# Seasandwpy/viso

Measured on AMD Instinct MI355X. Metric: stereo frames/sec at 1242x375 grey, 1/2/4/8 GPUs; pose RMSE vs reference, higher is better.
Workload: dtype f64

## Files before the change

### viso_amd/csrc/common.hpp

```cpp
#pragma once

#include <hip/hip_runtime.h>

#include <cstddef>
#include <cstdint>
#include <cstdio>

namespace viso {

constexpr int kLevels = 4;
constexpr int kHalfPatch = 4;
constexpr int kPatch = 64;
constexpr int kMaxWidth = 4096;

struct PyrGeom {
    int w[kLevels], h[kLevels];
    size_t off[kLevels];
    size_t bytes;
    size_t slot;
};

inline PyrGeom make_geom(int w, int h) {
    PyrGeom g{};
    size_t off = 0;
// ... 36 lines not shown
    return ((const __attribute__((address_space(1))) uint8_t*)p)[i];
}
__device__ inline uint8_t ld_global_u8_off(const uint8_t* base, uint32_t off) {
    return ((const __attribute__((address_space(1))) uint8_t*)base)[off];
}
__device__ inline int ld_u8_or0(const uint8_t* p, long long n, long long i) {
    const bool in = i >= 0 && i < n;
    const int v = ld_global_u8(p, in ? i : 0);
    return in ? v : 0;
}
__device__ inline uint8_t ld_lds_u8(const uint8_t* p, int i) {
    return ((const __attribute__((address_space(3))) uint8_t*)p)[i];
}
__device__ inline void st_lds_u8(uint8_t* p, int i, uint8_t v) {
    ((__attribute__((address_space(3))) uint8_t*)p)[i] = v;
}

__device__ inline double sample_px(const uint8_t* __restrict__ img, int w, int h, double x,
                                   double y) {
    const long long n = (long long)w * (long long)h;
    const bool finite = (x > -1e9 && x < 1e9 && y > -1e9 && y < 1e9);
    long long base = finite ? (long long)(int)y * (long long)w + (long long)(int)x : -(1LL << 40);
    double d0 = (double)ld_u8_or0(img, n, base);
    double d1 = (double)ld_u8_or0(img, n, base + 1);
    double d2 = (double)ld_u8_or0(img, n, base + w);
    double d3 = (double)ld_u8_or0(img, n, base + w + 1);
    double xx = x - floor(x);
    double yy = y - floor(y);
    return double((1 - xx) * (1 - yy) * d0 + xx * (1 - yy) * d1 + (1 - xx) * yy * d2 +
                  xx * yy * d3);
}

__device__ inline void gradient_px(const uint8_t* __restrict__ img, int w, int h, double u,
                                   double v, double& gx, double& gy) {
    gx = 0.5 * (sample_px(img, w, h, u + 1, v) - sample_px(img, w, h, u - 1, v));
    gy = 0.5 * (sample_px(img, w, h, u, v + 1) - sample_px(img, w, h, u, v - 1));
}

__device__ inline double wave_tree_sum(double v) {
#pragma unroll
    for (int off = 1; off < 64; off <<= 1) v = v + __shfl_xor(v, off, 64);
    return v;
}

template <int CTRL>
__device__ inline double dpp_f64(double v) {
    const long long b = __double_as_longlong(v);
    const int lo = __builtin_amdgcn_mov_dpp((int)(b & 0xffffffffLL), CTRL, 0xF, 0xF, true);
    const int hi = __builtin_amdgcn_mov_dpp((int)(b >> 32), CTRL, 0xF, 0xF, true);
    return __longlong_as_double(((long long)hi << 32) | (unsigned int)lo);
}

__device__ inline int wave_id() { return __builtin_amdgcn_readfirstlane((int)(threadIdx.x >> 6)); }

__device__ inline double uniform_f64(double v) {
    const long long b = __double_as_longlong(v);
    const int lo = __builtin_amdgcn_readfirstlane((int)(b & 0xffffffffLL));
    const int hi = __builtin_amdgcn_readfirstlane((int)(b >> 32));
    return __longlong_as_double(((long long)hi << 32) | (unsigned int)lo);
}

__device__ inline double readlane_f64(double v, int lane) {
    const long long b = __double_as_longlong(v);
    const int lo = __builtin_amdgcn_readlane((int)(b & 0xffffffffLL), lane);
    const int hi = __builtin_amdgcn_readlane((int)(b >> 32), lane);
    return __longlong_as_double(((long long)hi << 32) | (unsigned int)lo);
}

__device__ inline void permlane16_swap_f64(double a, double b, double& ra, double& rb) {
    const long long x = __double_as_longlong(a), y = __double_as_longlong(b);
    const auto lo = __builtin_amdgcn_permlane16_swap((unsigned)(x & 0xffffffffLL),
                                                     (unsigned)(y & 0xffffffffLL), false, false);
    const auto hi = __builtin_amdgcn_permlane16_swap((unsigned)(x >> 32), (unsigned)(y >> 32), false,
                                                     false);
    ra = __longlong_as_double(((long long)hi[0] << 32) | lo[0]);
    rb = __longlong_as_double(((long long)hi[1] << 32) | lo[1]);
}

__device__ inline void permlane32_swap_f64(double a, double b, double& ra, double& rb) {
    const long long x = __double_as_longlong(a), y = __double_as_longlong(b);
    const auto lo = __builtin_amdgcn_permlane32_swap((unsigned)(x & 0xffffffffLL),
                                                     (unsigned)(y & 0xffffffffLL), false, false);
    const auto hi = __builtin_amdgcn_permlane32_swap((unsigned)(x >> 32), (unsigned)(y >> 32), false,
                                                     false);
    ra = __longlong_as_double(((long long)hi[0] << 32) | lo[0]);
    rb = __longlong_as_double(((long long)hi[1] << 32) | lo[1]);
}

__device__ inline double wave_tree_sum_dpp(double v) {
    v = v + dpp_f64<0xB1>(v);
    v = v + dpp_f64<0x4E>(v);
    v = v + dpp_f64<0x141>(v);
    v = v + dpp_f64<0x140>(v);
    double a, b;
    permlane16_swap_f64(v, v, a, b);
    v = a + b;
    permlane32_swap_f64(v, v, a, b);
    return a + b;
}

__device__ inline double dsel(bool c, double a, double b) { return c ? a : b; }

__device__ inline void wave_tree_sum3(double a, double b, double c, double& ra, double& rb, double& rc) {
    const int lane = threadIdx.x & 63;
    const bool b0 = lane & 1, b1 = lane & 2, b2 = lane & 4, b3 = lane & 8;
    const double p = (b0 ? b : a) + dpp_f64<0xB1>(b0 ? a : b);
    const double q = (b0 ? 0.0 : c) + dpp_f64<0xB1>(b0 ? c : 0.0);
    double v = (b1 ? q : p) + dpp_f64<0x4E>(b1 ? p : q);
    const double r4 = dpp_f64<0x114>(v), l4 = dpp_f64<0x104>(v);
    v = v + dsel(b2, r4, l4);
    v = v + dpp_f64<0x128>(v);
    double x, y;
    permlane16_swap_f64(v, v, x, y);
    v = x + y;
    permlane32_swap_f64(v, v, x, y);
    v = x + y;
    ra = readlane_f64(v, 0);
    rb = readlane_f64(v, 1);
    rc = readlane_f64(v, 2);
}

__device__ inline void wave_tree_sum3_desc(double a, double b, double c, double& ra, double& rb, double& rc) {
    const int lane = threadIdx.x & 63;
    const bool b2 = lane & 4, b3 = lane & 8;
    double x, y;
    permlane32_swap_f64(a, b, x, y);
    const double ab = x + y;
    permlane32_swap_f64(c, c, x, y);
    const double cc = x + y;
    permlane16_swap_f64(ab, cc, x, y);
    double v = x + y;
    v = v + dpp_f64<0x128>(v);
    v = v + dpp_f64<0x124>(v);
    v = v + dpp_f64<0x4E>(v);
    v = v + dpp_f64<0xB1>(v);
    ra = readlane_f64(v, 0);
    rb = readlane_f64(v, 32);
    rc = readlane_f64(v, 16);
}


template <int CTRL>
__device__ inline double dpp_or0(double v) {
    return dpp_f64<CTRL>(v);
}

__device__ inline double swizzle_xor16_f64(double v) {
    const long long b = __double_as_longlong(v);
    const int lo = __builtin_amdgcn_ds_swizzle((int)(b & 0xffffffffLL), 0x401F);
    const int hi = __builtin_amdgcn_ds_swizzle((int)(b >> 32), 0x401F);
    return __longlong_as_double(((long long)hi << 32) | (unsigned int)lo);
}

__device__ inline double reduce_scatter_28_paired(const double* a, int* value_index) {
    const int lane = threadIdx.x & 63;
    const bool b0 = lane & 1, b1 = lane & 2, b2 = lane & 4, b3 = lane & 8, b5 = lane & 32;
    double c[7];
#pragma unroll
    for (int k = 0; k < 7; ++k) {
        const double send = dsel(b0, a[k], a[7 + k]);
        const double keep = dsel(b0, a[7 + k], a[k]);
        c[k] = keep + dpp_f64<0xB1>(send);
    }
    double d[4];
#pragma unroll
    for (int k = 0; k < 4; ++k) {
        const double hi = k < 3 ? c[4 + k] : 0.0;
        const double send = dsel(b1, c[k], hi);
        const double keep = dsel(b1, hi, c[k]);
        d[k] = keep + dpp_f64<0x4E>(send);
    }
    double e[2];
#pragma unroll
    for (int k = 0; k < 2; ++k) {
        const double send = dsel(b2, d[k], d[2 + k]);
        const double keep = dsel(b2, d[2 + k], d[k]);
        const double recv = dsel(b2, dpp_f64<0x114>(send), dpp_f64<0x104>(send));
        e[k] = keep + recv;
    }
    const double send = dsel(b3, e[0], e[1]);
    const double keep = dsel(b3, e[1], e[0]);
    double f = keep + dpp_f64<0x128>(send);
    double ra, rb;
    permlane16_swap_f64(f, f, ra, rb);
    f = ra + rb;
    const int local = (b1 ? 4 : 0) + (b2 ? 2 : 0) + (b3 ? 1 : 0);
    *value_index = local >= 7 ? -1 : (b5 ? 14 : 0) + (b0 ? 7 : 0) + local;
    return f;
}

__device__ inline double reduce_scatter_28(const double* v, int* value_index) {
    const int lane = threadIdx.x & 63;
    const bool b0 = lane & 1, b1 = lane & 2, b2 = lane & 4, b3 = lane & 8, b4 = lane & 16;
    double a[14];
#pragma unroll
    for (int k = 0; k < 14; ++k) {
        const double send = dsel(b0, v[k], v[14 + k]);
        const double keep = dsel(b0, v[14 + k], v[k]);
        a[k] = keep + dpp_f64<0xB1>(send);
    }
    double c[7];
#pragma unroll
    for (int k = 0; k < 7; ++k) {
        const double send = dsel(b1, a[k], a[7 + k]);
        const double keep = dsel(b1, a[7 + k], a[k]);
        c[k] = keep + dpp_f64<0x4E>(send);
    }
    double d[4];
#pragma unroll
    for (int k = 0; k < 4; ++k) {
        const double hi = k < 3 ? c[4 + k] : 0.0;
        const double send = dsel(b2, c[k], hi);
        const double keep = dsel(b2, hi, c[k]);
        const double recv = dsel(b2, dpp_f64<0x114>(send), dpp_f64<0x104>(send));
        d[k] = keep + recv;
    }
    double e[2];
#pragma unroll
    for (int k = 0; k < 2; ++k) {
        const double send = dsel(b3, d[k], d[2 + k]);
        const double keep = dsel(b3, d[2 + k], d[k]);
        const double recv = dpp_f64<0x128>(send);
        e[k] = keep + recv;
    }
    double ra, rb;
    permlane16_swap_f64(e[0], e[1], ra, rb);
    double f = ra + rb;
    permlane32_swap_f64(f, f, ra, rb);
    f = ra + rb;
    *value_index = (b0 ? 14 : 0) + (b1 ? 7 : 0) + (b2 ? 4 : 0) + (b3 ? 2 : 0) + (b4 ? 1 : 0);
    const int local = (b2 ? 4 : 0) + (b3 ? 2 : 0) + (b4 ? 1 : 0);
    if (local >= 7) *value_index = -1;
    return f;
}

__device__ inline double reduce_scatter_28_desc(const double* v, int* value_index) {
    const int lane = threadIdx.x & 63;
    const bool b0 = lane & 1, b1 = lane & 2, b2 = lane & 4, b3 = lane & 8, b4 = lane & 16, b5 = lane & 32;
    double a[14];
#pragma unroll
    for (int k = 0; k < 14; ++k) {
        double ra, rb;
        permlane32_swap_f64(v[k], v[14 + k], ra, rb);
        a[k] = ra + rb;
    }
    double c[7];
#pragma unroll
    for (int k = 0; k < 7; ++k) {
        double ra, rb;
        permlane16_swap_f64(a[k], a[7 + k], ra, rb);
        c[k] = ra + rb;
    }
    double d[4];
#pragma unroll
    for (int k = 0; k < 4; ++k) {
        const double hi = k < 3 ? c[4 + k] : 0.0;
        const double send = dsel(b3, c[k], hi);
        const double keep = dsel(b3, hi, c[k]);
        const double recv = dpp_f64<0x128>(send);
        d[k] = keep + recv;
    }
    double e[2];
#pragma unroll
    for (int k = 0; k < 2; ++k) {
        const double send = dsel(b2, d[k], d[2 + k]);
        const double keep = dsel(b2, d[2 + k], d[k]);
        const double recv = dsel(b2, dpp_f64<0x114>(send), dpp_f64<0x104>(send));
        e[k] = keep + recv;
    }
    const double send = dsel(b1, e[0], e[1]);
    const double keep = dsel(b1, e[1], e[0]);
    double f = keep + dpp_f64<0x4E>(send);
    f = f + dpp_f64<0xB1>(f);
    const int local = (b3 ? 4 : 0) + (b2 ? 2 : 0) + (b1 ? 1 : 0);
    *value_index = (b0 || local >= 7) ? -1 : (b5 ? 14 : 0) + (b4 ? 7 : 0) + local;
    return f;
}

template <int CTRL>
__device__ inline float dpp_f32(float v) {
    return __int_as_float(__builtin_amdgcn_mov_dpp(__float_as_int(v), CTRL, 0xF, 0xF, true));
}

__device__ inline void permlane16_swap_f32(float a, float b, float& ra, float& rb) {
    const auto r = __builtin_amdgcn_permlane16_swap((unsigned)__float_as_int(a), (unsigned)__float_as_int(b),
                                                    false, false);
    ra = __int_as_float((int)r[0]);
    rb = __int_as_float((int)r[1]);
}

__device__ inline void permlane32_swap_f32(float a, float b, float& ra, float& rb) {
    const auto r = __builtin_amdgcn_permlane32_swap((unsigned)__float_as_int(a), (unsigned)__float_as_int(b),
                                                    false, false);
    ra = __int_as_float((int)r[0]);
    rb = __int_as_float((int)r[1]);
}

__device__ inline float reduce_scatter_28_f32(const float* v, int* value_index) {
    const int lane = threadIdx.x & 63;
    const bool b0 = lane & 1, b1 = lane & 2, b2 = lane & 4, b3 = lane & 8, b4 = lane & 16;
    float a[14];
#pragma unroll
    for (int k = 0; k < 14; ++k) {
        const float send = b0 ? v[k] : v[14 + k];
        const float keep = b0 ? v[14 + k] : v[k];
        a[k] = keep + dpp_f32<0xB1>(send);
    }
    float c[7];
#pragma unroll
    for (int k = 0; k < 7; ++k) {
        const float send = b1 ? a[k] : a[7 + k];
        const float keep = b1 ? a[7 + k] : a[k];
        c[k] = keep + dpp_f32<0x4E>(send);
    }
    float d[4];
#pragma unroll
    for (int k = 0; k < 4; ++k) {
        const float hi = k < 3 ? c[4 + k] : 0.0f;
        const float send = b2 ? c[k] : hi;
        const float keep = b2 ? hi : c[k];
        const float r4 = dpp_f32<0x114>(send), l4 = dpp_f32<0x104>(send);
        const float recv = b2 ? r4 : l4;
        d[k] = keep + recv;
    }
    float e[2];
#pragma unroll
    for (int k = 0; k < 2; ++k) {
        const float send = b3 ? d[k] : d[2 + k];
        const float keep = b3 ? d[2 + k] : d[k];
        e[k] = keep + dpp_f32<0x128>(send);
    }
    float ra, rb;
    permlane16_swap_f32(e[0], e[1], ra, rb);
    float f = ra + rb;
    permlane32_swap_f32(f, f, ra, rb);
    f = ra + rb;
    *value_index = (b0 ? 14 : 0) + (b1 ? 7 : 0) + (b2 ? 4 : 0) + (b3 ? 2 : 0) + (b4 ? 1 : 0);
    const int local = (b2 ? 4 : 0) + (b3 ? 2 : 0) + (b4 ? 1 : 0);
    if (local >= 7) *value_index = -1;
    return f;
}
// ... 70 lines not shown
```

### viso_amd/csrc/direct.hip

```cpp
#include <algorithm>
#include <cstring>

#include "device_math.hpp"
#include "direct_solve.hpp"
#include "kernels.hpp"

#ifdef VISO_PROBE
constexpr int kPRing = 4096;
constexpr int kPSt = 24;
__device__ unsigned long long g_plog[kPRing][kPSt];
__device__ unsigned long long g_pexit[kPRing];
constexpr int kPRingB = 512;
__device__ unsigned long long g_pblk[kPRingB][256][4];
__device__ unsigned long long g_pwave[kPRingB][256][16];
#ifdef VISO_PROBE_PT
constexpr int kPtRing = 128, kPtBlocks = 32, kPtStamps = 5;
__device__ unsigned long long g_ppt[kPtRing][kPtBlocks][16][kPtStamps];
#define PPT(k)                                                                                       \
    do {                                                                                             \
        if (blockIdx.x < kPtBlocks && (threadIdx.x & 63) == 0)                                       \
            g_ppt[a.probe_seq & (kPtRing - 1)][blockIdx.x][threadIdx.x >> 6][(k)] =                  \
                __builtin_amdgcn_s_memrealtime();                                                    \
    } while (0)
#endif
#define PROBE_DECL()                                \
    __shared__ unsigned long long pst[kPSt];        \
    const unsigned long long probe_t0 = __builtin_amdgcn_s_memrealtime()
#define PST(k)                                                                       \
    do {                                                                             \
        if (blockIdx.x == 0 && (threadIdx.x & 63) == 0) pst[(k)] = __builtin_amdgcn_s_memrealtime(); \
    } while (0)
#else
#define PROBE_DECL()
#define PST(k)
#endif
#ifndef VISO_PROBE_PT
#define PPT(k) ((void)0)
#endif

namespace viso {

namespace {

constexpr int kSums = 28;
#ifndef VISO_DIRECT_WAVES
#define VISO_DIRECT_WAVES 12
#endif
constexpr int kWaves = VISO_DIRECT_WAVES;
constexpr int kThreads = kWaves * 64;
constexpr int kRigWaves = 16;
constexpr int kRigThreads = kRigWaves * 64;
constexpr int kMaxTiles = 256;
constexpr int kMaxTile = kMaxMapPoints / kMaxTiles;

inline int map_tile(int n, int groups) {
    int t = (n + groups - 1) / groups;
    return t < 1 ? 1 : (t > kMaxTile ? kMaxTile : t);
}
constexpr int kStats = 50;
constexpr int kStateStride = 8;
constexpr int kHdrBg = 1 << 17;

struct FramePair {
    FrameDev last;
    FrameDev cur;
    const double* pose_last;
};

struct LevelPair {
    const uint8_t* last;
    const uint8_t* cur;
    const double* pose_last;
};

__device__ inline LevelPair level_pair(const FramePair& fp, int lv) {
    return LevelPair{fp.last.l[lv], fp.cur.l[lv], fp.pose_last};
}

struct DirectArgs {
    FramePair fp;
    PyrDev g;
    Intrinsics K;
    const double* points;
    int n;
    const double* pose_seed;
    int level;
    int tile;
    int n_tiles;
    int split;
    DirectScratch s;
    double* stats;
    double* pose_out;
    double* log;
    int log_index;
    double* log_host;
    double* prev_log_host;
    int merged;
    int probe_seq;
    FramePair prev;
    double* prev_pose_out;
    double* prev_log;
    int prev_log_index;
    int* ready;
    int* prev_ready;
    double* flog;
};

__device__ inline void store_frame_pose(double* dst, const double* pose, int* ready) {
#pragma unroll
    for (int k = 0; k < 12; ++k) __hip_atomic_store(dst + k, pose[k], __ATOMIC_RELAXED, __HIP_MEMORY_SCOPE_AGENT);
    if (ready) {
        asm volatile("s_waitcnt vmcnt(0)" ::: "memory");
        __hip_atomic_store(ready, 1, __ATOMIC_RELAXED, __HIP_MEMORY_SCOPE_AGENT);
    }
}

__device__ inline void log_pose(double* log, double* log_host, int index, const double* pose) {
    if (!log || index < 0) return;
    for (int k = 0; k < 12; ++k) log[12 * (size_t)index + k] = pose[k];
    if (log_host)
        for (int k = 0; k < 12; ++k)
            __hip_atomic_store(log_host + 12 * (size_t)index + k, pose[k], __ATOMIC_RELAXED, __HIP_MEMORY_SCOPE_SYSTEM);
}

__device__ inline void log_frame(double* flog, int index, const SolveLds& L) {
    if (!flog || index < 0) return;
    flog[4 * (size_t)index + 0] = (double)L.ngood;
    flog[4 * (size_t)index + 1] = L.cost;
}

__device__ inline void tile_range(const DirectArgs& a, int b, int* first, int* cnt) {
    if (a.split) {
        const int f = (int)(((long long)b * a.n) / a.n_tiles);
        *first = f;
        *cnt = (int)(((long long)(b + 1) * a.n) / a.n_tiles) - f;
    } else {
        *first = b * a.tile;
        *cnt = a.tile;
    }
}

__device__ inline void d_pixel_d_xi(const Intrinsics& K, const double* pose, const double* P,
                                    double scale, double* J) {
    double Pc[3];
    mat3_vec(pose, P, Pc);
    Pc[0] = Pc[0] + pose[9];
    Pc[1] = Pc[1] + pose[10];
    Pc[2] = Pc[2] + pose[11];
    const double x = Pc[0], y = Pc[1], z = Pc[2];
    const double fx = K.fx * scale, fy = K.fy * scale;
    const double zz = z * z, xy = x * y;
    J[0] = fx / z;
    J[1] = 0;
    J[2] = -fx * x / zz;
    J[3] = -fx * xy / zz;
    J[4] = fx + fx * x * x / zz;
    J[5] = -fx * y / z;
    J[6] = 0;
    J[7] = fy / z;
    J[8] = -fy * y / zz;
    J[9] = -fy - fy * y * y / zz;
    J[10] = fy * xy / zz;
    J[11] = fy * x / z;
}

struct RefSample {
    double P[3];
    double ur, vr;
    double xx, yy;
    double lval;
    int t0, t1, t2, t3;
    bool ok;
};

__device__ inline void ref_project(const DirectArgs& a, const LevelPair& fp, int lv, int i, RefSample& r) {
    const int lane = threadIdx.x & 63;
    const int px = (lane >> 3) - 4, py = (lane & 7) - 4;
    const double scale = kScale[lv];
    const int w = a.g.w[lv], h = a.g.h[lv];
    r.P[0] = a.points[3 * i];
    r.P[1] = a.points[3 * i + 1];
    r.P[2] = a.points[3 * i + 2];
    project_px(fp.pose_last, a.K, r.P, scale, r.ur, r.vr);
    const double hp = 4.0;
    r.ok = inside_px(r.ur - hp, r.vr - hp, w, h) && inside_px(r.ur + hp, r.vr + hp, w, h);
    const double x = r.ur + px, y = r.vr + py;
    r.xx = x - floor(x);
    r.yy = y - floor(y);
}

__device__ inline void ref_taps(const DirectArgs& a, const LevelPair& fp, int lv, RefSample& r,
                                unsigned* raw = nullptr) {
    const int lane = threadIdx.x & 63;
    const int px = (lane >> 3) - 4, py = (lane & 7) - 4;
    const int w = a.g.w[lv], h = a.g.h[lv];
    const double x = r.ur + px, y = r.vr + py;
    const uint8_t* img = fp.last;
    const long long n = (long long)w * (long long)h;
    const long long base = r.ok ? (long long)(int)y * (long long)w + (long long)(int)x : -(1LL << 40);
    if (raw) {
        const long long i0 = base, i1 = base + 1, i2 = base + w, i3 = base + w + 1;
        const bool in0 = i0 >= 0 && i0 < n, in1 = i1 >= 0 && i1 < n, in2 = i2 >= 0 && i2 < n,
                   in3 = i3 >= 0 && i3 < n;
        r.t0 = ld_global_u8(img, in0 ? i0 : 0);
        r.t1 = ld_global_u8(img, in1 ? i1 : 0);
        r.t2 = ld_global_u8(img, in2 ? i2 : 0);
// ... 497 lines not shown
}

__device__ inline float fast_lval(uint32_t t, double ur, double vr);

template <bool LV16>
__device__ inline void pf_store(int j, bool ref, const PfPoint& q, PfLds& pf) {
    const int lane = threadIdx.x & 63;
    if (ref) {
        const uint32_t t0 = q.tin & 1u ? (uint32_t)q.r.t0 : 0u, t1 = q.tin & 2u ? (uint32_t)q.r.t1 : 0u;
        const uint32_t t2 = q.tin & 4u ? (uint32_t)q.r.t2 : 0u, t3 = q.tin & 8u ? (uint32_t)q.r.t3 : 0u;
        pf.taps[j][lane] = t0 | (t1 << 8) | (t2 << 16) | (t3 << 24);
    }
    if (LV16) pf.lv16[j][lane] = (_Float16)(q.r.ok ? fast_lval(pf.taps[j][lane], q.r.ur, q.r.vr) : 0.0f);
    if (q.c.on) win_store(pf.win[j], q.c);
    if (lane == 0) {
        pf.P[j][0] = q.r.P[0];
        pf.P[j][1] = q.r.P[1];
        pf.P[j][2] = q.r.P[2];
        pf.ur[j] = ref ? q.r.ur : 0.0;
        pf.vr[j] = ref ? q.r.vr : 0.0;
        pf.ok[j] = (ref && q.r.ok) ? 1 : 0;
        pf.cw[j][0] = q.c.x0;
        pf.cw[j][1] = q.c.y0;
        pf.cw[j][2] = q.c.on ? 1 : 0;
    }
}

template <bool LV16 = false>
__device__ void prefetch_tile(const DirectArgs& a, int lv, int b, const double* pred, const double* pose_last,
                              bool ref, int first, int stride, PfLds& pf, const FramePair* fpair = nullptr) {
    LevelPair fp = level_pair(fpair ? *fpair : a.fp, lv);
    fp.pose_last = pose_last;
    int p0, T;
    tile_range(a, b, &p0, &T);
    for (int j = first; j < T; j += 2 * stride) {
        const int j2 = j + stride;
        const int i0 = p0 + j, i1 = p0 + j2;
        const bool v0 = i0 < a.n, v1 = j2 < T && i1 < a.n;
        PfPoint q0{}, q1{};
        if (v0) pf_project(a, fp, lv, i0, pred, ref, q0);
        if (v1) pf_project(a, fp, lv, i1, pred, ref, q1);
        if (v0) pf_issue(a, fp, lv, ref, q0);
        if (v1) pf_issue(a, fp, lv, ref, q1);
        if (v0) pf_store<LV16>(j, ref, q0, pf);
        if (v1) pf_store<LV16>(j2, ref, q1, pf);
    }
}

__device__ inline void pf_ref(const PfLds& pf, int j, RefSample& r) {
    const int lane = threadIdx.x & 63;
    const int px = (lane >> 3) - 4, py = (lane & 7) - 4;
    r.P[0] = pf.P[j][0];
    r.P[1] = pf.P[j][1];
    r.P[2] = pf.P[j][2];
    r.ur = pf.ur[j];
    r.vr = pf.vr[j];
    r.ok = pf.ok[j] != 0;
    const uint32_t t = pf.taps[j][lane];
    r.t0 = (int)(t & 0xff);
    r.t1 = (int)((t >> 8) & 0xff);
    r.t2 = (int)((t >> 16) & 0xff);
    r.t3 = (int)(t >> 24);
    const double x = r.ur + px, y = r.vr + py;
    r.xx = x - floor(x);
    r.yy = y - floor(y);
    ref_finish(r);
}

__device__ inline void merged_ref(const DirectArgs& a, const LevelPair& fp, int lv, const PfLds& pf, int j,
                                  RefSample& r) {
    const int lane = threadIdx.x & 63;
    const int px = (lane >> 3) - 4, py = (lane & 7) - 4;
    const int w = a.g.w[lv], h = a.g.h[lv];
    r.P[0] = pf.P[j][0];
    r.P[1] = pf.P[j][1];
    r.P[2] = pf.P[j][2];
    project_px(fp.pose_last, a.K, r.P, kScale[lv], r.ur, r.vr);
    const double hp = 4.0;
    r.ok = inside_px(r.ur - hp, r.vr - hp, w, h) && inside_px(r.ur + hp, r.vr + hp, w, h);
    const double x = r.ur + px, y = r.vr + py;
    r.xx = x - floor(x);
    r.yy = y - floor(y);
    r.t0 = r.t1 = r.t2 = r.t3 = 0;
    if (!r.ok) return;
    const long long base = (long long)(int)y * (long long)w + (long long)(int)x;
    const double xp = pf.ur[j] + px, yp = pf.vr[j] + py;
    const long long bp = pf.ok[j] ? (long long)(int)yp * (long long)w + (long long)(int)xp : -(1LL << 40);
#ifdef VISO_PROBE_PFB
    {
        const unsigned long long rl = __ballot(base != bp);
        if (lane == 0) {
            PFB_ADD(5);
            if (rl) PFB_ADD(4);
        }
    }
#endif
    if (__builtin_expect(base == bp, 1)) {
        const uint32_t t = pf.taps[j][lane];
        r.t0 = (int)(t & 0xff);
        r.t1 = (int)((t >> 8) & 0xff);
        r.t2 = (int)((t >> 16) & 0xff);
        r.t3 = (int)(t >> 24);
    } else {
        const uint8_t* img = fp.last;
        const long long n = (long long)w * (long long)h;
        r.t0 = ld_u8_or0(img, n, base);
        r.t1 = ld_u8_or0(img, n, base + 1);
        r.t2 = ld_u8_or0(img, n, base + w);
        r.t3 = ld_u8_or0(img, n, base + w + 1);
    }
}

__device__ inline void scalar_pass(const DirectArgs& a, int lv, const double* cur_pose, const PfLds& pf, int first,
                                   int T, int helper, SpLds& sp) {
    const int lane = threadIdx.x & 63;
    const bool act = lane < kSpPerHelper * kSpLanes;
    const int p = act ? lane / kSpLanes : kSpPerHelper - 1;
    const int k = act ? lane - kSpLanes * p : kSpLanes - 1;
    const int j = kSpPerHelper * helper + p;
    const bool valid = act && j < T && first + j < a.n;
    const double scale = kScale[lv];
    const int w = a.g.w[lv], h = a.g.h[lv];
    const double P[3] = {pf.P[j][0], pf.P[j][1], pf.P[j][2]};
    const double q = quotient_select(a.K, cur_pose, P, scale, k);
    const double Q0 = bperm_f64(q, kSpLanes * p), Q1 = bperm_f64(q, kSpLanes * p + 1);
    const double uc = scale * (Q0 * a.K.fx + a.K.cx);
    const double vc = scale * (Q1 * a.K.fy + a.K.cy);
    const double hp = 4.0;
    const bool in = inside_px(uc - hp, vc - hp, w, h) && inside_px(uc + hp, vc + hp, w, h);
    const int fu = (int)floor(uc), fv = (int)floor(vc);
    const bool whole = patch_in_window(pf.cw[j][2] != 0, pf.cw[j][0], pf.cw[j][1], fu, fv);
    const int cls = !in ? kClsOut : !whole ? kClsSample : patch_one_binade(uc, vc) ? kClsShared : kClsStraddle;
    const double xx = uc - floor(uc), yy = vc - floor(vc);
    const double w00 = (1 - xx) * (1 - yy), w10 = xx * (1 - yy), w01 = (1 - xx) * yy, w11 = xx * yy;
    const bool shared = cls == kClsShared;
    if (valid) {
        sp.v[j][k] = q;
        if (k == 0) {
            double2* v2 = reinterpret_cast<double2*>(&sp.v[j][12]);
            v2[0] = make_double2(shared ? w00 : uc, shared ? w10 : vc);
            v2[1] = make_double2(w01, w11);
            *reinterpret_cast<int4*>(sp.cls[j]) = make_int4(cls, fu, fv, 0);
        }
    }
    __builtin_amdgcn_fence(__ATOMIC_RELEASE, "workgroup");
    if (valid && k == 0) __hip_atomic_store(&sp.ready[j], 1, __ATOMIC_RELAXED, __HIP_MEMORY_SCOPE_WORKGROUP);
}

constexpr unsigned kSrcHere = 0xffffffffu;

template <bool PAIRED>
__device__ inline size_t partial_index(int k, int b) {
    if (!PAIRED) return (size_t)k * kMaxTiles + b;
    const int h = k >= kSums / 2 ? 1 : 0;
    return (size_t)((((k - h * (kSums / 2)) * 4 + (b >> 6)) * 2 + h) * 64 + (b & 63));
}

template <bool FAST, bool LV16 = false, int W = kWaves, bool PAIRED = false>
__device__ void direct_tile_pf(const DirectArgs& a, const LevelPair& fp, int lv, const double* cur_pose, int b,
                               const PfLds& pf, bool merged, double* part, int* good, double* s_pts,
                               int* s_good, int* s_cnt = nullptr, double* s_qt = nullptr,
                               unsigned src_in = kSrcHere, SpLds* sp = nullptr) {
    const int wave = wave_id(), lane = threadIdx.x & 63;
    int first, T;
    tile_range(a, b, &first, &T);
    int good_cnt = 0;
    const unsigned src_lanes = FAST ? 0u : src_in != kSrcHere ? src_in : factored_sources();
    const bool sp_on = !FAST && W == kWaves && sp && s_cnt && T > kSpPoints - kSpHelpers && T <= kSpPoints;
    if (sp_on && wave >= kSpPoints) {
        __builtin_amdgcn_s_setprio(3);
        scalar_pass(a, lv, cur_pose, pf, first, T, wave - kSpPoints, *sp);
        __builtin_amdgcn_s_setprio(1);
    }
    for (int local = wave; local < T; local += W) {
        const int i = first + local;
        double f = 0.0;
        int idx = -1;
        bool ok = false;
        if (i < a.n) {
            RefSample r;
            if (merged) {
                merged_ref(a, fp, lv, pf, local, r);
                if (!FAST) ref_finish(r);
            } else if (!FAST) {
                pf_ref(pf, local, r);
            } else {
                r.P[0] = pf.P[local][0];
                r.P[1] = pf.P[local][1];
                r.P[2] = pf.P[local][2];
                r.ur = pf.ur[local];
                r.vr = pf.vr[local];
                r.ok = pf.ok[local] != 0;
                const uint32_t t = pf.taps[local][lane];
                r.t0 = (int)(t & 0xff);
                r.t1 = (int)((t >> 8) & 0xff);
                r.t2 = (int)((t >> 16) & 0xff);
                r.t3 = (int)(t >> 24);
            }
            CurWin cw;
            cw.x0 = pf.cw[local][0];
            cw.y0 = pf.cw[local][1];
            cw.on = pf.cw[local][2] != 0;
            if (FAST) {
                float ff = 0.0f;
                if (r.ok) {
                    const uint32_t t = (uint32_t)r.t0 | ((uint32_t)r.t1 << 8) | ((uint32_t)r.t2 << 16) |
                                       ((uint32_t)r.t3 << 24);
                    const float lval = (LV16 && !merged) ? (float)pf.lv16[local][lane] : fast_lval(t, r.ur, r.vr);
                    ok = direct_point_fast(a, fp, lv, cur_pose, r.P, lval, pf.win[local], cw, &ff, &idx);
                }
                f = (double)ff;
            } else if (sp_on) {
                ok = direct_point_sp(a, fp, lv, r, pf.win[local], cw, *sp, local, &f, &idx, src_lanes);
            } else {
                ok = direct_point_rs(a, fp, lv, cur_pose, r, pf.win[local], cw, &f, &idx, src_lanes,
                                     s_qt ? s_qt + 12 * wave : nullptr);
            }
        }
        if (!ok) {
            if (lane < kSums) s_pts[local * kSums + lane] = 0.0;
        } else if ((!FAST || lane < 32) && idx >= 0) {
            s_pts[local * kSums + idx] = f;
        }
        good_cnt += ok ? 1 : 0;
    }
    if (lane == 0 && good_cnt) atomicAdd(s_good, good_cnt);
#ifdef VISO_PROBE
    if (threadIdx.x == 0 && blockIdx.x < 256) g_pblk[a.probe_seq & (kPRingB - 1)][blockIdx.x][2] = __builtin_amdgcn_s_memrealtime();
    if (lane == 0 && blockIdx.x < 256 && wave < 15)
        g_pwave[a.probe_seq & (kPRingB - 1)][blockIdx.x][wave] = __builtin_amdgcn_s_memrealtime();
#endif
    if (s_cnt && T <= 16) {
        const int nw = T < W ? T : W;
        if (wave >= nw) return;
        int prev = 0;
        if (lane == 0)
            prev = __hip_atomic_fetch_add(s_cnt, 1, __ATOMIC_ACQ_REL, __HIP_MEMORY_SCOPE_WORKGROUP);
        prev = __builtin_amdgcn_readfirstlane(prev);
        if (prev != nw - 1) return;
        __builtin_amdgcn_fence(__ATOMIC_ACQUIRE, "workgroup");
        if (lane < kSums) {
            double v[16];
#pragma unroll
            for (int j = 0; j < 16; ++j) v[j] = j < T ? s_pts[j * kSums + lane] : 0.0;
#pragma unroll
            for (int st = 1; st < 16; st <<= 1)
#pragma unroll
                for (int j = 0; j < 16; j += 2 * st) v[j] = v[j] + v[j + st];
            double r = v[0] + 0.0;
            r = r + 0.0;
            part[partial_index<PAIRED>(lane, b)] = r;
        }
        if (lane == 0) good[b] = __hip_atomic_load(s_good, __ATOMIC_RELAXED, __HIP_MEMORY_SCOPE_WORKGROUP);
#ifdef VISO_PROBE
        if (lane == 0 && blockIdx.x < 256)
            g_pwave[a.probe_seq & (kPRingB - 1)][blockIdx.x][15] = __builtin_amdgcn_s_memrealtime();
#endif
        return;
    }
    __syncthreads();
    for (int k = wave; k < kSums; k += W) {
        const double v = lane < T ? s_pts[lane * kSums + k] : 0.0;
        const double r = wave_tree_sum_dpp(v);
        if (lane == 0) part[partial_index<PAIRED>(k, b)] = r;
    }
    if (threadIdx.x == 0) good[b] = *s_good;
    __syncthreads();
}

__device__ inline void state_to_pose(const double* st, double* pose) {
    double q[4] = {st[0], st[1], st[2], st[3]};
    quat_to_matrix(q, pose);
    pose[9] = st[4];
    pose[10] = st[5];
    pose[11] = st[6];
}


__device__ inline void load_partials(const double* __restrict__ part, const int* __restrict__ good,
                                     int n_tiles, double* v, int& gg) {
    const int t = threadIdx.x;
    if (t < n_tiles) {
#pragma unroll
        for (int k = 0; k < kSums; ++k) v[k] = part[(size_t)k * kMaxTiles + t];
        gg = good[t];
    } else {
#pragma unroll
        for (int k = 0; k < kSums; ++k) v[k] = 0.0;
        gg = 0;
    }
}

__device__ inline void load_partials_paired(const double* __restrict__ part, const int* __restrict__ good,
                                            int n_tiles, double* a, int& gg) {
    const int t = threadIdx.x;
    const int t0 = (t & ~63) + 2 * (t & 31);
    if (t0 < n_tiles) {
        const bool has1 = t0 + 1 < n_tiles;
        const double2* __restrict__ p2 = reinterpret_cast<const double2*>(part) + t;
#pragma unroll
        for (int k = 0; k < kSums / 2; ++k) {
            const double2 x = p2[(size_t)k * kMaxTiles];
            a[k] = x.x + (has1 ? x.y : 0.0);
        }
    } else {
#pragma unroll
        for (int k = 0; k < kSums / 2; ++k) a[k] = 0.0;
    }
    gg = t < n_tiles ? good[t] : 0;
}

__device__ inline void reduce_partials(const double* v, int gg, SolveLds& L) {
    const int t = threadIdx.x, wave = t >> 6, lane = t & 63;
    if (t < 256) {
        int idx;
        const double f = reduce_scatter_28(v, &idx);
        if (lane < 32 && idx >= 0) L.red[wave][idx] = f;
        const int g = wave_sum_int(gg);
        if (lane == 0) L.g[wave] = g;
    }
    __syncthreads();
    if (t < kSums) L.S[t] = (L.red[0][t] + L.red[1][t]) + (L.red[2][t] + L.red[3][t]);
    if (t == 0) L.ngood = (L.g[0] + L.g[1]) + (L.g[2] + L.g[3]);
    __syncthreads();
}

__device__ inline void lds_barrier() { asm volatile("s_waitcnt lgkmcnt(0)\n\ts_barrier" ::: "memory"); }

template <bool FAST>
__device__ void solve_continue(const DirectArgs& a, const FramePair& fpair, int lv, SolveLds& L,
                               double* stats, double* s_pose, double* s_pts, int* s_good, PfLds& pf) {
    const int t = threadIdx.x, wave = t >> 6;
    double* part = a.s.cont_part + (size_t)blockIdx.x * kMaxTiles * kSums;
    int* good = a.s.cont_good + (size_t)blockIdx.x * kMaxTiles;
    const LevelPair fp = level_pair(fpair, lv);
    for (int iter = 1; iter < 100 && L.cont; ++iter) {
        if (t == 0) state_to_pose(L.state, s_pose);
        __syncthreads();
        double pose[12];
#pragma unroll
        for (int k = 0; k < 12; ++k) pose[k] = s_pose[k];
        for (int b = 0; b < a.n_tiles; ++b) {
            if (t == 0) *s_good = 0;
            prefetch_tile(a, lv, b, pose, fpair.pose_last, true, wave, kWaves, pf, &fpair);
            __syncthreads();
            direct_tile_pf<FAST>(a, fp, lv, pose, b, pf, false, part, good, s_pts, s_good);
        }
        __threadfence_block();
        __syncthreads();
        double v[kSums];
        int gg = 0;
        if (t < 256) load_partials(part, good, a.n_tiles, v, gg);
        reduce_partials(v, gg, L);
        if (wave == 0) {
            if (FAST)
                solve_wave0_ldlt(L, iter, stats);
            else
                solve_wave0(L, iter, stats);
        }
        __syncthreads();
    }
}

__device__ inline void prefetch_point(const DirectArgs& a, int lv, int i, bool solve, int sl,
                                      RefSample& r, CurWin& cw) {
    ref_issue(a, level_pair(a.fp, lv), lv, i, r);
    double pred[12];
    if (!solve) {
        for (int k = 0; k < 12; ++k) pred[k] = a.pose_seed[k];
    } else {
        double sp[7];
        for (int k = 0; k < 7; ++k) sp[k] = a.s.state[sl * kStateStride + k];
        state_to_pose(sp, pred);
    }
    double up, vp;
    project_px(pred, a.K, r.P, kScale[lv], up, vp);
    win_issue(a.fp.cur.l[lv], a.g.w[lv], a.g.h[lv], up, vp, cw);
}

__device__ inline void after_solve(const DirectArgs& a, bool merged, SolveLds& L, double* s_last,
                                   double* s_pose) {
    if (merged) {
        state_to_pose(L.state, s_last);
        if (blockIdx.x == 0) {
            for (int k = 0; k < 7; ++k) a.s.state[kLevels * kStateStride + k] = L.state[k];
            if (a.prev_pose_out) store_frame_pose(a.prev_pose_out, s_last, a.prev_ready);
            log_pose(a.prev_log, a.prev_log_host, a.prev_log_index, s_last);
            log_frame(a.flog, a.prev_log_index, L);
        }
        double q[4];
        quat_from_matrix(s_last, q);
        for (int k = 0; k < 4; ++k) L.state[k] = q[k];
        L.state[4] = s_last[9];
        L.state[5] = s_last[10];
        L.state[6] = s_last[11];
    }
    state_to_pose(L.state, s_pose);
}

template <bool FAST, bool SP = false>
__global__ __launch_bounds__(kThreads, 4) void direct_level_kernel(const double* __restrict__ pre_part,
                                                                 const int* __restrict__ pre_good, int pre_hdr,
                                                                 DirectArgs a) {
    PROBE_DECL();
    __builtin_amdgcn_s_setprio(1);
    __shared__ SolveLds L;
    __shared__ double s_pose[12];
    __shared__ double s_last[12];
    __shared__ double s_pts[kMaxTile * kSums];
    __shared__ int s_good;
    __shared__ int s_cnt;
    __shared__ int s_arrive;
    __shared__ PfLds s_pf;
#ifndef VISO_NO_QT
    __shared__ __attribute__((aligned(16))) double s_qt[FAST ? 2 : kWaves * 12];
    double* const qt = FAST ? nullptr : s_qt;
#else
    double* const qt = nullptr;
#endif
    __shared__ __attribute__((aligned(16))) SpLds s_sp;
    const int lv = a.level;
    const bool merged = a.merged && lv == kLevels - 1;
    const int prev = lv + 1;
    const bool solve = prev < kLevels || merged;
    const int sl = merged ? 0 : prev;
    const int t = threadIdx.x, wave = t >> 6, lane = t & 63;
    const bool tiles = lv >= 0 && (int)blockIdx.x < a.n_tiles;
    double v[kSums / 2];
    int gg = 0;
    if (((pre_hdr >> 16) & 1) && t < 256) load_partials_paired(pre_part, pre_good, pre_hdr & 0xffff, v, gg);
    const bool pf_wave = !solve || (wave & 3) != 0;
    double st[7];
    if (t == 256 || (solve && tiles && pf_wave)) {
        if (!solve) {
            quat_from_matrix(a.pose_seed, st);
            st[4] = a.pose_seed[9];
            st[5] = a.pose_seed[10];
            st[6] = a.pose_seed[11];
        } else {
#pragma unroll
            for (int k = 0; k < 7; ++k) st[k] = a.s.state[sl * kStateStride + k];
        }
    }
    if (t == 0) {
        s_arrive = 0;
        s_good = 0;
        s_cnt = 0;
#ifdef VISO_PROBE
        for (int k = 0; k < kPSt; ++k) pst[k] = 0;
        pst[0] = probe_t0;
        if (blockIdx.x < 256) g_pblk[a.probe_seq & (kPRingB - 1)][blockIdx.x][0] = probe_t0;
#endif
    }
    if (SP && t >= kThreads - kSpPoints) s_sp.ready[kThreads - 1 - t] = 0;
    lds_barrier();
    if (wave == 0) PST(16);

    if (t == 256) {
        for (int k = 0; k < 7; ++k) {
            L.state[k] = st[k];
            L.best[k] = st[k];
        }
        L.cost = 0.0;
        L.last_cost = 0.0;
        L.cont = 0;
        asm volatile("s_waitcnt lgkmcnt(0)" ::: "memory");
        atomicAdd(&s_arrive, 1);
    }
    if (solve && t < 256) {
#ifdef VISO_PROBE
        asm volatile("s_waitcnt vmcnt(0)" ::: "memory");
        if (wave == 0) PST(17);
#endif
        int idx;
        const double f = reduce_scatter_28_paired(v, &idx);
        if (!(lane & 16) && idx >= 0) L.red[wave][idx] = f;
        const int g = wave_sum_int(gg);
        if (lane == 0) L.g[wave] = g;
        asm volatile("s_waitcnt lgkmcnt(0)" ::: "memory");
        if (wave == 0) PST(18);
        if (lane == 0) atomicAdd(&s_arrive, 1);
    }
    if (wave == 0) PST(1);

    const bool solver = solve && wave == 0;
    if (tiles && pf_wave) {
        double pred[12];
        if (!solve) {
            for (int k = 0; k < 12; ++k) pred[k] = a.pose_seed[k];
        } else {
#ifdef VISO_PROBE
            if (wave == 5) {
                asm volatile("s_waitcnt vmcnt(0)" ::: "memory");
                PST(20);
            }
#endif
            state_to_pose(st, pred);
        }
        const int first = solve ? wave - (wave >> 2) - 1 : wave;
        const int stride = solve ? kWaves - kWaves / 4 : kWaves;
        prefetch_tile(a, lv, blockIdx.x, pred, merged ? pred : a.fp.pose_last, true, first, stride, s_pf);
#ifdef VISO_PROBE
        asm volatile("s_waitcnt vmcnt(0) lgkmcnt(0)" ::: "memory");
        if (blockIdx.x == 0 && lane == 0) atomicMax(&pst[9], __builtin_amdgcn_s_memrealtime());
#endif
    }

    if (solver) {
        __builtin_amdgcn_s_setprio(3);
        while (__hip_atomic_load(&s_arrive, __ATOMIC_RELAXED, __HIP_MEMORY_SCOPE_WORKGROUP) < 5)
            __builtin_amdgcn_s_sleep(1);
        PST(19);
        if (lane < kSums) L.S[lane] = (L.red[0][lane] + L.red[1][lane]) + (L.red[2][lane] + L.red[3][lane]);
        if (lane == 0) L.ngood = (L.g[0] + L.g[1]) + (L.g[2] + L.g[3]);
        PST(2);
        double* stp = (a.stats && blockIdx.x == 0) ? a.stats + (size_t)kStats * sl : nullptr;
#ifdef VISO_PROBE
        unsigned long long stamps[5] = {probe_t0, probe_t0, probe_t0, probe_t0, probe_t0};
        if (FAST)
            solve_wave0_ldlt(L, 0, stp, stamps);
        else
            solve_wave0(L, 0, stp, stamps);
        if (blockIdx.x == 0 && lane == 0)
            for (int k = 0; k < 4; ++k) pst[3 + k] = stamps[k];
        if (blockIdx.x == 0 && lane == 0) pst[12] = stamps[4];
#else
        if (FAST)
            solve_wave0_ldlt(L, 0, stp);
        else
            solve_wave0(L, 0, stp);
#endif
        PST(7);
        __builtin_amdgcn_s_setprio(1);
    }
    if (!solve && wave == 0 && lane == 0) {
        while (__hip_atomic_load(&s_arrive, __ATOMIC_RELAXED, __HIP_MEMORY_SCOPE_WORKGROUP) < 1)
            __builtin_amdgcn_s_sleep(1);
    }
    if (wave == 0 && lane == 0 && !L.cont) after_solve(a, merged, L, s_last, s_pose);
    const unsigned src_lanes = FAST ? 0u : factored_sources();
    __syncthreads();
    if (__builtin_expect(solve && L.cont, 0)) {
        double* stp = (a.stats && blockIdx.x == 0) ? a.stats + (size_t)kStats * sl : nullptr;
        solve_continue<FAST>(a, merged ? a.prev : a.fp, sl, L, stp, s_pose, s_pts, &s_good, s_pf);
        if (t == 0) {
            after_solve(a, merged, L, s_last, s_pose);
            s_good = 0;
        }
        __syncthreads();
        if (tiles) {
            double pose[12];
#pragma unroll
            for (int k = 0; k < 12; ++k) pose[k] = s_pose[k];
            prefetch_tile(a, lv, blockIdx.x, pose, merged ? s_last : a.fp.pose_last, true, wave, kWaves, s_pf);
        }
        __syncthreads();
    }
    if (wave == 0) PST(8);
#ifdef VISO_PROBE
    if (t == 0 && blockIdx.x < 256) g_pblk[a.probe_seq & (kPRingB - 1)][blockIdx.x][1] = __builtin_amdgcn_s_memrealtime();
#endif
    const int out = lv >= 0 ? lv : kLevels;
    if (blockIdx.x == 0 && t == 0 && !merged) {
        for (int k = 0; k < 7; ++k) a.s.state[out * kStateStride + k] = L.state[k];
        if (lv < 0 && a.pose_out) {
            store_frame_pose(a.pose_out, s_pose, a.ready);
            log_pose(a.log, a.log_host, a.log_index, s_pose);
            log_frame(a.flog, a.log_index, L);
        }
    }
    if (blockIdx.x == 0 && t == 0 && merged)
        for (int k = 0; k < 7; ++k) a.s.state[lv * kStateStride + k] = L.state[k];
    if (tiles) {
        LevelPair fp = level_pair(a.fp, lv);
        if (merged) fp.pose_last = s_last;
        double pose[12];
#pragma unroll
        for (int k = 0; k < 12; ++k) pose[k] = s_pose[k];
        direct_tile_pf<FAST, false, kWaves, true>(a, fp, lv, pose, blockIdx.x, s_pf, merged,
                                                  a.s.part + (size_t)lv * kMaxTiles * kSums,
                                                  a.s.good + lv * kMaxTiles, s_pts, &s_good, &s_cnt, qt,
                                                  src_lanes, SP ? &s_sp : nullptr);
    }
#ifdef VISO_PROBE
    __syncthreads();
    const unsigned long long t_exit = __builtin_amdgcn_s_memrealtime();
    const int slot = a.probe_seq & (kPRing - 1);
    if (t == 0 && blockIdx.x < 256) g_pblk[a.probe_seq & (kPRingB - 1)][blockIdx.x][3] = t_exit;
    if (blockIdx.x == 0 && t == 0) {
        pst[11] = t_exit;
        pst[15] = (unsigned long long)(lv + 1) | ((unsigned long long)merged << 8) |
                  ((unsigned long long)a.n_tiles << 16);
        for (int k = 0; k < kPSt; ++k) g_plog[slot][k] = pst[k];
    }
#endif
}

constexpr int kRigTiles = kMaxTiles;

__device__ __host__ inline int rig_reduce_waves(int n_tiles) { return n_tiles <= 64 ? 1 : n_tiles <= 128 ? 2 : 4; }

struct RigCamArgs {
    DirectArgs d;
    const double* Ad;
    double E[12];
};

struct RigArgs {
    RigCamArgs cam[kMaxRigCams];
    int n_cams;
    int tile_off[kMaxRigCams + 1];
    int level;
    double* state;
    const double* seed;
    double* stats;
    double* pose_out;
    double* log;
    int log_index;
    double* cam_last;
    int merged;
    double* prev_pose_out;
    double* prev_log;
    int prev_log_index;
};

__device__ inline void rig_compose(const double* E, const double* T, double* out) {
#pragma unroll
    for (int i = 0; i < 3; ++i) {
#pragma unroll
// ... 696 lines not shown
```

Before: 22130.

## Reorganize paired partial layout for per-lane tree reduction of 16 tiles

Changes the global layout of per-tile partial sums so that each of 56 lanes per wave loads 16 tiles' worth of a pair of sums and reduces them in registers with a serial tree. Only two DPP steps then finish the reduction, replacing the longer cross-lane reduce-scatter sequence that used permlane and many select ops. This cuts cross-lane shuffle work in the solver's preamble. In exchange, each lane issues more (conditional) global loads and holds a 16-element double2 array, which raises register pressure.

Result: faster. 22860 (median of 6 runs) (+3.3%).

```diff
diff --git a/viso_amd/csrc/common.hpp b/viso_amd/csrc/common.hpp
--- a/viso_amd/csrc/common.hpp
+++ b/viso_amd/csrc/common.hpp
@@ -212,41 +212,19 @@
     return __longlong_as_double(((long long)hi << 32) | (unsigned int)lo);
 }
 
-__device__ inline double reduce_scatter_28_paired(const double* a, int* value_index) {
-    const int lane = threadIdx.x & 63;
-    const bool b0 = lane & 1, b1 = lane & 2, b2 = lane & 4, b3 = lane & 8, b5 = lane & 32;
-    double c[7];
-#pragma unroll
-    for (int k = 0; k < 7; ++k) {
-        const double send = dsel(b0, a[k], a[7 + k]);
-        const double keep = dsel(b0, a[7 + k], a[k]);
-        c[k] = keep + dpp_f64<0xB1>(send);
-    }
-    double d[4];
-#pragma unroll
-    for (int k = 0; k < 4; ++k) {
-        const double hi = k < 3 ? c[4 + k] : 0.0;
-        const double send = dsel(b1, c[k], hi);
-        const double keep = dsel(b1, hi, c[k]);
-        d[k] = keep + dpp_f64<0x4E>(send);
-    }
-    double e[2];
-#pragma unroll
-    for (int k = 0; k < 2; ++k) {
-        const double send = dsel(b2, d[k], d[2 + k]);
-        const double keep = dsel(b2, d[2 + k], d[k]);
-        const double recv = dsel(b2, dpp_f64<0x114>(send), dpp_f64<0x104>(send));
-        e[k] = keep + recv;
-    }
-    const double send = dsel(b3, e[0], e[1]);
-    const double keep = dsel(b3, e[1], e[0]);
-    double f = keep + dpp_f64<0x128>(send);
-    double ra, rb;
-    permlane16_swap_f64(f, f, ra, rb);
-    f = ra + rb;
-    const int local = (b1 ? 4 : 0) + (b2 ? 2 : 0) + (b3 ? 1 : 0);
-    *value_index = local >= 7 ? -1 : (b5 ? 14 : 0) + (b0 ? 7 : 0) + local;
-    return f;
+__device__ inline double reduce_tree16_pairs(double2* x) {
+    const bool b0 = threadIdx.x & 1;
+#pragma unroll
+    for (int st = 1; st < 16; st <<= 1)
+#pragma unroll
+        for (int j = 0; j < 16; j += 2 * st) {
+            x[j].x = x[j].x + x[j + st].x;
+            x[j].y = x[j].y + x[j + st].y;
+        }
+    const double send = dsel(b0, x[0].x, x[0].y);
+    const double keep = dsel(b0, x[0].y, x[0].x);
+    const double c = keep + dpp_f64<0xB1>(send);
+    return c + dpp_f64<0x4E>(c);
 }
 
 __device__ inline double reduce_scatter_28(const double* v, int* value_index) {
diff --git a/viso_amd/csrc/direct.hip b/viso_amd/csrc/direct.hip
--- a/viso_amd/csrc/direct.hip
+++ b/viso_amd/csrc/direct.hip
@@ -52,6 +52,7 @@
 constexpr int kRigThreads = kRigWaves * 64;
 constexpr int kMaxTiles = 256;
 constexpr int kMaxTile = kMaxMapPoints / kMaxTiles;
+constexpr int kTreeLanes = kSums / 2 * 4;
 
 inline int map_tile(int n, int groups) {
     int t = (n + groups - 1) / groups;
@@ -855,8 +856,7 @@
 template <bool PAIRED>
 __device__ inline size_t partial_index(int k, int b) {
     if (!PAIRED) return (size_t)k * kMaxTiles + b;
-    const int h = k >= kSums / 2 ? 1 : 0;
-    return (size_t)((((k - h * (kSums / 2)) * 4 + (b >> 6)) * 2 + h) * 64 + (b & 63));
+    return (size_t)((((b >> 6) * 16 + (b & 15)) * kTreeLanes + ((k >> 1) * 4 + ((b >> 4) & 3))) * 2 + (k & 1));
 }
 
 template <bool FAST, bool LV16 = false, int W = kWaves, bool PAIRED = false>
@@ -994,21 +994,15 @@
     }
 }
 
-__device__ inline void load_partials_paired(const double* __restrict__ part, const int* __restrict__ good,
-                                            int n_tiles, double* a, int& gg) {
-    const int t = threadIdx.x;
-    const int t0 = (t & ~63) + 2 * (t & 31);
-    if (t0 < n_tiles) {
-        const bool has1 = t0 + 1 < n_tiles;
-        const double2* __restrict__ p2 = reinterpret_cast<const double2*>(part) + t;
-#pragma unroll
-        for (int k = 0; k < kSums / 2; ++k) {
-            const double2 x = p2[(size_t)k * kMaxTiles];
-            a[k] = x.x + (has1 ? x.y : 0.0);
-        }
-    } else {
-#pragma unroll
-        for (int k = 0; k < kSums / 2; ++k) a[k] = 0.0;
+__device__ inline void load_partials_tree16(const double* __restrict__ part, const int* __restrict__ good,
+                                            int n_tiles, double2* x, int& gg) {
+    const int t = threadIdx.x, lane = t & 63;
+    const int m = lane < kTreeLanes ? n_tiles - ((t & ~63) + 16 * (lane & 3)) : 0;
+    const double2* __restrict__ p2 = reinterpret_cast<const double2*>(part) + (size_t)(t >> 6) * 16 * kTreeLanes + lane;
+#pragma unroll
+    for (int j = 0; j < 16; ++j) {
+        x[j] = make_double2(0.0, 0.0);
+        if (j < m) x[j] = p2[j * kTreeLanes];
     }
     gg = t < n_tiles ? good[t] : 0;
 }
@@ -1129,9 +1123,9 @@
     const int sl = merged ? 0 : prev;
     const int t = threadIdx.x, wave = t >> 6, lane = t & 63;
     const bool tiles = lv >= 0 && (int)blockIdx.x < a.n_tiles;
-    double v[kSums / 2];
+    double2 v[16];
     int gg = 0;
-    if (((pre_hdr >> 16) & 1) && t < 256) load_partials_paired(pre_part, pre_good, pre_hdr & 0xffff, v, gg);
+    if (((pre_hdr >> 16) & 1) && t < 256) load_partials_tree16(pre_part, pre_good, pre_hdr & 0xffff, v, gg);
     const bool pf_wave = !solve || (wave & 3) != 0;
     double st[7];
     if (t == 256 || (solve && tiles && pf_wave)) {
@@ -1175,9 +1169,8 @@
         asm volatile("s_waitcnt vmcnt(0)" ::: "memory");
         if (wave == 0) PST(17);
 #endif
-        int idx;
-        const double f = reduce_scatter_28_paired(v, &idx);
-        if (!(lane & 16) && idx >= 0) L.red[wave][idx] = f;
+        const double f = reduce_tree16_pairs(v);
+        if (lane < kTreeLanes && !(lane & 2)) L.red[wave][2 * (lane >> 2) + (lane & 1)] = f;
         const int g = wave_sum_int(gg);
         if (lane == 0) L.g[wave] = g;
         asm volatile("s_waitcnt lgkmcnt(0)" ::: "memory");
```
